# lars-frogner/Impact

Hardware: AMD Instinct MI355X
Metric: voxels stepped/sec + remesh tris/sec, 512^3 grid, 1/2/4/8 MI355X (higher is better)
Workload: dtype i8 voxels, f32 SDF/mesh arithmetic, f64 moments; 1 GPU; config-2 SDF asteroid x2.05 -> 502^3 grid = 512^3 stored voxels (32768 chunks); parallelism=single GPU, voxels_per_gpu=134217728, regions=1, triangles=1813104

## Files before the change

impact_amd/csrc/ivx_api.hip:

```cpp
#include <algorithm>
#include <array>
#include <functional>
#include <cmath>
#include <atomic>
#include <chrono>
#include <cstring>
#include <limits>
#include <map>
#include <unordered_map>
#include <new>
#include <vector>

#include <type_traits>

#include <dlfcn.h>

#include "ivx_internal.hpp"

static thread_local char g_error[512] = "";

void ivx_set_error(const char* fmt, ...) {
    va_list ap;
    va_start(ap, fmt);
    vsnprintf(g_error, sizeof(g_error), fmt, ap);
// ... 602 lines not shown
        g->result_host = nullptr;
    }
    void* ptrs[] = {g->arena, g->positions, g->normals, g->indices, g->index_materials, g->vertex_materials, g->submeshes, g->dev_scratch, g->prog_nodes,
                    g->samp_len, g->samp_ops, g->pairs_dev, g->samp_super, g->probe_points, g->probe_chunk, g->probe_entries};
    for (void* p : ptrs)
        if (p) (void)hipFree(p);
    if (g->host_scratch) (void)hipHostFree(g->host_scratch);
    if (g->result_host) (void)hipHostFree(g->result_host);
    if (g->ev_ready)
        for (int i = 0; i < 2 * IVX_N_TIMED_STAGES; ++i) (void)hipEventDestroy(g->ev[i]);
    delete g;
}

int ivx_grid_upload_dense(ivx_grid* g, const int8_t* sdf, const uint8_t* type, size_t n_voxels) {
    IVX_REQUIRE(g && sdf && type, IVX_ERR_INVALID, "ivx_grid_upload_dense: null argument");
    IVX_REQUIRE(n_voxels == g->n_vox, IVX_ERR_INVALID, "ivx_grid_upload_dense: expected %zu voxels, got %zu", g->n_vox, n_voxels);
    int rc;
    if ((rc = h2d(g, g->sdf, sdf, g->n_vox))) return rc;
    if ((rc = h2d(g, g->type, type, g->n_vox))) return rc;
    if ((rc = ivx_launch_classify(g))) return rc;
    g->mesh_valid = 0;
    g->mesh_built = 0;
    g->occ_ref_valid = 0;
    g->bbox_valid = 0;
    g->regions_valid = 0;
    IVX_HIP_CHECK(ivx_stream_sync(g->ctx->stream));
    return IVX_OK;
}

int ivx_grid_download_dense(ivx_grid* g, int8_t* sdf, uint8_t* type, uint8_t* flags, uint8_t* local_labels, ivx_chunk_info* info, size_t n_voxels) {
// ... 43 lines not shown
        case 5: return g->rparent;
#ifdef IVX_WG_TRACE
        case 6: return g->chunk_moments;
#endif
        case 7: return g->samp_len;
        case 8: return g->samp_ops;
        case 10: return g->sn_hard;
        case 9: return ivx_sn_hard_count(g);
        default: return nullptr;
    }
}

int ivx_sdf_sample(ivx_grid* g, const ivx_sdf_processed_node* nodes, size_t n_nodes, uint32_t stack_size, const uint32_t grid_shape[3],
                   const float shifted_grid_center[3], uint8_t voxel_type) {
    IVX_REQUIRE(g && grid_shape && shifted_grid_center, IVX_ERR_INVALID, "ivx_sdf_sample: null argument");
    IVX_REQUIRE(n_nodes == 0 || nodes, IVX_ERR_INVALID, "ivx_sdf_sample: null node array");
    for (int d = 0; d < 3; ++d) {
        const uint32_t cap = (d == 0 ? g->gx : g->cc[d]) * 16u;
        IVX_REQUIRE(grid_shape[d] <= cap, IVX_ERR_INVALID, "ivx_sdf_sample: grid shape %u exceeds the chunk grid (%u voxels) along axis %d", grid_shape[d], cap, d);
    }
    int depth = 0, max_depth = 0;
    for (size_t i = 0; i < n_nodes; ++i) {
        const uint32_t k = nodes[i].kind;
        IVX_REQUIRE(k <= 9, IVX_ERR_INVALID, "ivx_sdf_sample: unsupported node kind %u", k);
        IVX_REQUIRE(k != 6 || nodes[i].reserved[1] <= 255u, IVX_ERR_INVALID, "ivx_sdf_sample: noise node with more than 255 octaves");
        if (k <= 2) max_depth = std::max(max_depth, ++depth);
        else if (k >= 7) {
            IVX_REQUIRE(depth >= 2, IVX_ERR_INVALID, "ivx_sdf_sample: malformed node program (combination without two operands)");
            --depth;
        } else if (k == 5 || k == 6) {
// ... 11 lines not shown
    }
    rc = ivx_launch_sdf_sample(g, static_cast<const ivx_sdf_processed_node*>(g->dev_scratch), (uint32_t)n_nodes, (uint32_t)max_depth, grid_shape,
                               shifted_grid_center, voxel_type, 0u, false, ivx_sdf_has_noise(nodes, n_nodes));
    if (rc) return rc;
    g->mesh_valid = 0;
    g->mesh_built = 0;
    g->occ_ref_valid = 0;
    g->bbox_valid = 0;
    g->regions_valid = 0;
    IVX_HIP_CHECK(ivx_stream_sync(g->ctx->stream));
    return IVX_OK;
}

int ivx_derive_state(ivx_grid* g) {
    IVX_REQUIRE(g, IVX_ERR_INVALID, "ivx_derive_state: null grid");
    int rc = ivx_launch_derive(g, 0);
    if (rc) return rc;
    g->mesh_valid = 0;
    g->regions_valid = 0;
    IVX_HIP_CHECK(ivx_stream_sync(g->ctx->stream));
    return IVX_OK;
}

int ivx_occupied_ranges(ivx_grid* g, uint32_t out[12]) {
    IVX_REQUIRE(g && out, IVX_ERR_INVALID, "ivx_occupied_ranges: null argument");
    IVX_REQUIRE(g->bbox_valid, IVX_ERR_STATE, "ivx_occupied_ranges: the chunk boxes come from the derive sweep (call ivx_derive_state first)");
    uint32_t* d = g->rscalar + 16;
    int rc;
    if ((rc = ivx_launch_occupied(g, d))) return rc;
    uint32_t raw[12];
    if ((rc = d2h(g, raw, d, 12 * sizeof(uint32_t)))) return rc;
    ivx_occupied_from_raw(g, raw, out);
    memcpy(g->occ_ref, out, sizeof(g->occ_ref));
    g->occ_ref_valid = 1;
    return IVX_OK;
}

int ivx_remesh(ivx_grid* g, ivx_mesh_counts* out) {
    IVX_REQUIRE(g && out, IVX_ERR_INVALID, "ivx_remesh: null argument");
    int rc;
    if ((rc = ivx_launch_sn_count(g))) return rc;
    if ((rc = ivx_launch_sn_scan(g))) return rc;
    uint32_t totals[3];
    if ((rc = d2h(g, totals, g->chunk_offsets + 2 * (size_t)g->n_chunks, sizeof(totals)))) return rc;
    if ((rc = ensure_mesh_capacity(g, totals[0], totals[1], totals[2]))) return rc;
    if (totals[1] > 0 && (rc = ivx_launch_sn_emit(g))) return rc;
    g->mesh_counts.n_vertices = totals[0];
    g->mesh_counts.n_indices = totals[1];
    g->mesh_counts.n_submeshes = totals[2];
    g->mesh_counts.reserved = 0;
    g->mesh_valid = 1;
    g->mesh_built = 1;
    g->mesh_serial += 1;
    *out = g->mesh_counts;
// ... 3 lines not shown

static void ivx_edit_state_free(struct ivx_edit_state* e);
struct ivx_edit_state;
static ivx_edit_state* edit_state(ivx_grid* g);
static bool edit_needs_lookup(ivx_grid* g, uint32_t chunk, uint32_t out3[3]);
static int edit_sync_upload(ivx_grid* g, const void* src, size_t bytes, void* d_dst);
static void edit_sync_mark(ivx_grid* g, int pending);
static int edit_sync_pending(ivx_grid* g);
static bool edit_sync_drained_take(ivx_grid* g);

static int edit_early_needs(ivx_grid* g, const char* who, std::vector<uint32_t>& list);
static int edit_sync_stage(ivx_grid* g, const void* src, size_t bytes, void** dev_view);
static int edit_sync_stage_done(ivx_grid* g);
static int mesh_sync_enqueue(ivx_grid* g, const uint8_t* invalidated_chunks, const char* who) {
    IVX_REQUIRE(g, IVX_ERR_INVALID, "%s: null argument", who);
    ivx_many_other_context other_(g->ctx);
    IVX_REQUIRE(!edit_sync_pending(g), IVX_ERR_STATE, "%s: a sync of this object is in flight (ivx_mesh_sync_collect first)", who);
    IVX_REQUIRE(g->mesh_built, IVX_ERR_STATE, "ivx_mesh_sync: there is no mesh to synchronise (call ivx_remesh first)");
    IVX_REQUIRE(g->regions_valid, IVX_ERR_STATE, "ivx_mesh_sync: derived state must be current (the edit ops leave it so)");
    IVX_REQUIRE(g->x_off == 0 && g->gx == g->cc[0] && !g->has_ghost[0] && !g->has_ghost[1], IVX_ERR_STATE,
                "ivx_mesh_sync: not available on a slab of a decomposed grid");
    int rc;
    static const bool trace_ = getenv("IVX_MANY_TRACE") != nullptr;
    static thread_local double acc_[6];
    static thread_local int calls_ = 0;
    auto tp_ = std::chrono::steady_clock::now();
    auto lap_ = [&](int slot) {
        if (!trace_) return;
        const auto t = std::chrono::steady_clock::now();
        acc_[slot] += 1e-3 * (double)std::chrono::duration_cast<std::chrono::nanoseconds>(t - tp_).count();
// ... 296 lines not shown

static int densities_on_device(ivx_grid* g, const float densities[256], const float** d_out) {
    if (g->has_dens && memcmp(g->dens_host, densities, sizeof(g->dens_host)) == 0) {
        *d_out = g->dens_dev;
        return IVX_OK;
    }
    if (!g->dens_call) IVX_HIP_CHECK(hipMalloc(reinterpret_cast<void**>(&g->dens_call), 256 * sizeof(float)));
    int rc = h2d(g, g->dens_call, densities, 256 * sizeof(float));
    if (rc) return rc;
    *d_out = g->dens_call;
    return IVX_OK;
}

int ivx_inertia(ivx_grid* g, const float densities[256], ivx_moments* out) {
    IVX_REQUIRE(g && densities && out, IVX_ERR_INVALID, "ivx_inertia: null argument");
    double* out_dev = g->partials + g->partial_blocks * 10;
    int rc;
    const float* d_dens = nullptr;
    if ((rc = densities_on_device(g, densities, &d_dens))) return rc;
    if ((rc = ivx_launch_inertia(g, d_dens, out_dev, 0))) return rc;
    if ((rc = d2h(g, out->m64, out_dev, 10 * sizeof(double)))) return rc;
    for (int i = 0; i < 10; ++i) out->m32[i] = (float)out->m64[i];
    out->reserved[0] = out->reserved[1] = 0;
    return IVX_OK;
}

int ivx_label_regions(ivx_grid* g, uint32_t* region_count) {
    IVX_REQUIRE(g && region_count, IVX_ERR_INVALID, "ivx_label_regions: null argument");
    int rc;
    if ((rc = ivx_launch_ccl_local(g, 0))) return rc;
    if ((rc = ivx_launch_ccl_merge(g))) return rc;
    if ((rc = ivx_launch_ccl_resolve(g))) return rc;
    uint32_t sc[2];
    if ((rc = d2h(g, sc, g->rscalar, sizeof(sc)))) return rc;
    IVX_REQUIRE((sc[1] & 1u) == 0, IVX_ERR_CAPACITY,
                "ivx_label_regions: a chunk has more than 254 local regions (the reference's CHUNK_MAX_REGIONS limit, split_detection.rs:145-157)");
    g->region_count = sc[0];
    g->regions_valid = 1;
    *region_count = sc[0];
    return IVX_OK;
}

int ivx_region_labels_download(ivx_grid* g, uint32_t* labels, size_t n_voxels) {
// ... 76 lines not shown
}
static int rederive_collect(ivx_grid* g) {
    ivx_step_result res;
    const int rc = ivx_voxel_step_collect(g, &res);
    if (rc) return rc;
    g->mesh_valid = 0;
    return IVX_OK;
}
static int rederive(ivx_grid* g) {
    const int rc = rederive_enqueue(g);
    return rc ? rc : rederive_collect(g);
}

int ivx_split_off_smallest_region(ivx_grid* parent, ivx_grid** child, uint32_t origin_offset_in_parent[3], int* outcome, ivx_region_desc* moved) {
    IVX_REQUIRE(parent && child && origin_offset_in_parent && outcome, IVX_ERR_INVALID, "ivx_split_off_smallest_region: null argument");
    *child = nullptr;
    *outcome = 0;
    IVX_REQUIRE(parent->regions_valid, IVX_ERR_STATE, "ivx_split_off_smallest_region: call ivx_label_regions first");
    IVX_REQUIRE(parent->x_off == 0 && parent->gx == parent->cc[0] && !parent->has_ghost[0] && !parent->has_ghost[1], IVX_ERR_STATE,
                "ivx_split_off_smallest_region: not available on a slab of a decomposed grid");
    if (parent->region_count < 2) return IVX_OK;
    int rc;
    if (!parent->has_dens) {
        float ones[256];
        for (float& x : ones) x = 1.0f;
        if ((rc = h2d(parent, parent->dens_dev, ones, sizeof(ones)))) return rc;
        memcpy(parent->dens_host, ones, sizeof(ones));
        parent->has_dens = 1;
    }
    std::vector<ivx_region_desc> d;
// ... 44 lines not shown
        return rc;
    }
    if (c && (rc = rederive(c))) {
        ivx_grid_destroy(c);
        return rc;
    }
    *child = c;
    *outcome = c ? 1 : 2;
    return IVX_OK;
}

static int step_enqueue(ivx_grid* g, uint32_t stages, const uint16_t* slab_nbr_ids, void* slab_record, uint32_t part = 3u);
static int ivx_step_collect_launch(ivx_grid* g);
int ivx_split_off_all(ivx_grid* parent, size_t cap, ivx_grid** children, uint32_t* origins3, int* outcomes, ivx_region_desc* moved, size_t* n_out) {
    IVX_REQUIRE(parent && n_out && (cap == 0 || (children && origins3 && outcomes)), IVX_ERR_INVALID, "ivx_split_off_all: null argument");
    *n_out = 0;
    IVX_REQUIRE(parent->regions_valid, IVX_ERR_STATE, "ivx_split_off_all: call ivx_label_regions first");
    IVX_REQUIRE(parent->x_off == 0 && parent->gx == parent->cc[0] && !parent->has_ghost[0] && !parent->has_ghost[1], IVX_ERR_STATE,
                "ivx_split_off_all: not available on a slab of a decomposed grid");
    if (parent->region_count < 2) return IVX_OK;
    const size_t n = parent->region_count - 1u;
    *n_out = n;
    IVX_REQUIRE(n <= cap, IVX_ERR_CAPACITY, "ivx_split_off_all: %zu split-offs exceed capacity %zu", n, cap);
    int rc;
    hipStream_t s = parent->ctx->stream;
    float ones[256];
    for (float& x : ones) x = 1.0f;
    if (!parent->has_dens) {
        if ((rc = h2d(parent, parent->dens_dev, ones, sizeof(ones)))) return rc;
        memcpy(parent->dens_host, ones, sizeof(ones));
// ... 164 lines not shown
        if ((rc = ivx_launch_split_repack(c, single, off))) {
            ivx_grid_destroy(single);
            return rc;
        }
        ivx_grid_destroy(c);
        c = single;
        *pc = c;
        for (int q = 0; q < 3; ++q) origin[q] += off[q];
    }
    return rederive(c);
}

int ivx_clip_polyhedron(ivx_grid* parent, const float* planes4, size_t n_planes, const float aabb[6], int copy, ivx_grid** child,
                        uint32_t origin_offset_in_parent[3], int* outcome) {
    IVX_REQUIRE(parent && planes4 && aabb && child && origin_offset_in_parent && outcome, IVX_ERR_INVALID, "ivx_clip_polyhedron: null argument");
    *child = nullptr;
    *outcome = 0;
    IVX_REQUIRE(n_planes >= 1 && n_planes <= 64, IVX_ERR_CAPACITY, "ivx_clip_polyhedron: 1..64 planes supported, got %zu", n_planes);
    IVX_REQUIRE(parent->regions_valid, IVX_ERR_STATE, "ivx_clip_polyhedron: the object needs its derived state (ivx_derive_state + ivx_label_regions)");
    IVX_REQUIRE(parent->x_off == 0 && parent->gx == parent->cc[0] && !parent->has_ghost[0] && !parent->has_ghost[1], IVX_ERR_STATE,
                "ivx_clip_polyhedron: not available on a slab of a decomposed grid");
    int rc;
    uint32_t* d_occ = parent->rscalar + 16;
    if ((rc = ivx_launch_occupied(parent, d_occ))) return rc;
    uint32_t occ[12], occ_raw[12];
    if ((rc = d2h(parent, occ_raw, d_occ, sizeof(occ_raw)))) return rc;
    ivx_occupied_from_raw(parent, occ_raw, occ);
    if (occ[1] == 0) return IVX_OK;
    uint32_t lo[3], cc[3];
    for (int q = 0; q < 3; ++q) {
// ... 16 lines not shown
        ivx_grid_destroy(c);
        return rc;
    }
    if ((rc = complete_extracted(parent, &c, origin_offset_in_parent))) {
        if (c) ivx_grid_destroy(c);
        return rc;
    }
    *child = c;
    *outcome = c ? 1 : 2;
    return IVX_OK;
}

int ivx_copy_polyhedra(ivx_grid* parent, const float* planes4, const uint32_t* plane_counts, const float* aabbs6, size_t n_sets, ivx_grid** children,
                       uint32_t* origins3, int* outcomes) {
    IVX_REQUIRE(parent && planes4 && plane_counts && aabbs6 && children && origins3 && outcomes, IVX_ERR_INVALID, "ivx_copy_polyhedra: null argument");
    IVX_REQUIRE(parent->regions_valid, IVX_ERR_STATE, "ivx_copy_polyhedra: the object needs its derived state (ivx_derive_state + ivx_label_regions)");
    IVX_REQUIRE(parent->x_off == 0 && parent->gx == parent->cc[0] && !parent->has_ghost[0] && !parent->has_ghost[1], IVX_ERR_STATE,
                "ivx_copy_polyhedra: not available on a slab of a decomposed grid");
    for (size_t f = 0; f < n_sets; ++f) {
        children[f] = nullptr;
        outcomes[f] = 0;
        IVX_REQUIRE(plane_counts[f] >= 1 && plane_counts[f] <= 64, IVX_ERR_CAPACITY, "ivx_copy_polyhedra: 1..64 planes per polyhedron, set %zu has %u", f, plane_counts[f]);
    }
    if (n_sets == 0) return IVX_OK;
    int rc;
    hipStream_t s = parent->ctx->stream;
    uint32_t* d_occ = parent->rscalar + 16;
    if ((rc = ivx_launch_occupied(parent, d_occ))) return rc;
    uint32_t occ[12], occ_raw[12];
    if ((rc = d2h(parent, occ_raw, d_occ, sizeof(occ_raw)))) return rc;
// ... 240 lines not shown
    int rc = ensure_pinned(&e->pinned_up, &e->pinned_up_bytes, bytes);
    if (rc) return rc;
    if (e->pinned_up_bytes != had || !e->pinned_up_dev) IVX_HIP_CHECK(hipHostGetDevicePointer(&e->pinned_up_dev, e->pinned_up, 0));
    memcpy(e->pinned_up, src, bytes);
    *dev_view = e->pinned_up_dev;
    return IVX_OK;
}
static int edit_sync_stage_done(ivx_grid* g) {
    (void)g;
    return IVX_OK;
}

static int absorb_enqueue(ivx_grid* g, const char* who, int capsule, const float center[3], const float seg[3], float influence_radius, float shape_radius,
                          const float densities[256]) {
    IVX_REQUIRE(g && center && densities && (seg || !capsule), IVX_ERR_INVALID, "%s: null argument", who);
    ivx_many_other_context other_(g->ctx);
    IVX_REQUIRE(influence_radius >= 0.0f && shape_radius >= 0.0f, IVX_ERR_INVALID, "%s: negative radius", who);
    IVX_REQUIRE(g->regions_valid, IVX_ERR_STATE, "%s: derived state and regions must be current (ivx_derive_state + ivx_label_regions)", who);
    IVX_REQUIRE(g->x_off == 0 && g->gx == g->cc[0] && !g->has_ghost[0] && !g->has_ghost[1], IVX_ERR_STATE, "%s: not available on a slab of a decomposed grid",
                who);
    ivx_edit_state* e = edit_state(g);
    IVX_REQUIRE(e, IVX_ERR_CAPACITY, "%s: out of host memory", who);
    IVX_REQUIRE(!e->pending, IVX_ERR_STATE, "%s: an edit of this object is in flight (ivx_absorb_collect first)", who);
    int rc;
    uint32_t occ[12];
    if ((rc = reference_occupied(g, occ))) return rc;
    int32_t vlo[3], vhi[3];
    uint32_t lo[3], cc[3];
    e->nothing = 0;
    for (int d = 0; d < 3; ++d) {
// ... 71 lines not shown
    e->early_armed = 0, e->early_taken = 0;
    if (e->staged && g->early_needs_on) {
        e->early_seq += 1u;
        g->post1_needs_early = reinterpret_cast<uint32_t*>(static_cast<char*>(e->pinned_dev) + e->off_early);
        g->post1_needs_counter = reinterpret_cast<uint32_t*>(base + e->off_cnt) + 2;
        g->post1_needs_bell = reinterpret_cast<uint32_t*>(static_cast<char*>(e->pinned_dev) + e->off_bell);
        g->post1_needs_seq = e->early_seq;
        *reinterpret_cast<volatile uint32_t*>(static_cast<char*>(e->pinned) + e->off_bell) = 0u;
        e->early_armed = 1;
    }
    {
        const uint32_t keep = g->stage_timing_off;
        g->stage_timing_off = 0xFFFFFFFFu;
        g->preset_fresh |= IVX_SCRATCH_REGIONS;
        g->regions_labelled_locally = 1;
        rc = ivx_voxel_step_enqueue(g, IVX_STAGE_REGIONS);
        g->regions_labelled_locally = 0;
        g->stage_timing_off = keep;
        if (rc) return rc;
    }
    if (e->staged) {
        g->gather_copy_src = reinterpret_cast<const uint32_t*>(base);
        g->gather_copy_dst = static_cast<uint32_t*>(e->pinned_dev);
        g->gather_copy_words = (uint32_t)(((e->early_armed ? e->off_needs : e->total) + 3) / 4);
    }
    e->pending = 1;
    return IVX_OK;
}

static int absorb_collect(ivx_grid* g, const char* who, ivx_absorb_result* out, uint32_t* emptied_by_type, uint8_t* invalidated_chunks) {
    IVX_REQUIRE(g && out, IVX_ERR_INVALID, "%s: null argument", who);
// ... 1012 lines not shown
             if ((r = ivx_launch_mutual_pass(q.a, q.b, &p.pass[0], nullptr, d_offsets, list_dev + out_offsets[i], counts[i], 1))) return r;
             return ivx_launch_mutual_pass(q.b, q.a, &p.pass[1], nullptr, d_offsets + p.wg_a, list_dev + out_offsets[i], counts[i], 1);
         })))
        return rc;
    IVX_HIP_CHECK(ivx_stream_sync(s));
    memcpy(out, c->pinned_scratch, run * sizeof(ivx_contact));
    return IVX_OK;
}

int ivx_absorb_mutual(ivx_grid* a, const float rotation_a[4], const float translation_a[3], const float densities_a[256], ivx_grid* b, const float rotation_b[4],
                      const float translation_b[3], const float densities_b[256], float smoothness, ivx_absorb_result* out_a, ivx_absorb_result* out_b,
                      uint8_t* invalidated_chunks_a, uint8_t* invalidated_chunks_b) {
    const char* who = "ivx_absorb_mutual";
    IVX_REQUIRE(a && b && rotation_a && translation_a && densities_a && rotation_b && translation_b && densities_b && out_a && out_b, IVX_ERR_INVALID,
                "%s: null argument", who);
    IVX_REQUIRE(a != b && a->ctx == b->ctx, IVX_ERR_INVALID, "%s: two different objects of one context are needed", who);
    IVX_REQUIRE(smoothness >= 0.0f, IVX_ERR_INVALID, "%s: negative smoothness", who);
    for (ivx_grid* g : {a, b}) {
        IVX_REQUIRE(g->regions_valid, IVX_ERR_STATE, "%s: derived state and regions must be current (ivx_derive_state + ivx_label_regions)", who);
        IVX_REQUIRE(g->x_off == 0 && g->gx == g->cc[0] && !g->has_ghost[0] && !g->has_ghost[1], IVX_ERR_STATE,
                    "%s: not available on a slab of a decomposed grid", who);
    }
    memset(out_a, 0, sizeof(*out_a));
    memset(out_b, 0, sizeof(*out_b));
    if (invalidated_chunks_a) memset(invalidated_chunks_a, 0, a->n_chunks);
    if (invalidated_chunks_b) memset(invalidated_chunks_b, 0, b->n_chunks);
    int rc;
    uint32_t occ_a[12], occ_b[12];
    if ((rc = reference_occupied(a, occ_a))) return rc;
    if ((rc = reference_occupied(b, occ_b))) return rc;
// ... 164 lines not shown
    g->vt_noise_freq = noise_frequency;
    g->vt_type_freq = voxel_type_frequency;
    g->vt_seed = seed;
    return IVX_OK;
}

int ivx_grid_set_densities(ivx_grid* g, const float densities[256]) {
    IVX_REQUIRE(g && densities, IVX_ERR_INVALID, "ivx_grid_set_densities: null argument");
    memcpy(g->dens_host, densities, sizeof(g->dens_host));
    if (!ivx_many_upload(g->ctx, g, g->dens_dev, g->dens_host, sizeof(g->dens_host)))
        IVX_HIP_CHECK(ivx_memcpy_async(g->dens_dev, g->dens_host, sizeof(g->dens_host), hipMemcpyHostToDevice, g->ctx->stream));
    g->has_dens = 1;
    return IVX_OK;
}

static int ensure_pairs(ivx_grid* g);
static int step_enqueue(ivx_grid* g, uint32_t stages, const uint16_t* slab_nbr_ids, void* slab_record, uint32_t part) {
    IVX_REQUIRE(g, IVX_ERR_INVALID, "ivx_voxel_step_enqueue: null grid");
    const bool front = (part & 1u) != 0u, back = (part & 2u) != 0u;
    ivx_many_other_context other_(g->ctx);
    IVX_REQUIRE(!(stages & IVX_STAGE_SAMPLE) || g->prog_n > 0, IVX_ERR_STATE, "ivx_voxel_step: no SDF program resident (ivx_grid_set_sdf_program)");
    IVX_REQUIRE(!(stages & IVX_STAGE_INERTIA) || g->has_dens, IVX_ERR_STATE, "ivx_voxel_step: no densities resident (ivx_grid_set_densities)");
    hipStream_t s = g->ctx->stream;
    g->ahead_unordered_ok = g->pending_stages == 0;
    g->results_in_block = 0;
    if (!g->ev_ready) {
        for (int i = 0; i < 2 * IVX_N_TIMED_STAGES; ++i) IVX_HIP_CHECK(hipEventCreate(&g->ev[i]));
        g->ev_ready = 1;
    }
    if (!g->result_host) {
        IVX_HIP_CHECK(hipHostMalloc(reinterpret_cast<void**>(&g->result_host), 64 * sizeof(uint32_t), hipHostMallocMapped));
        memset(g->result_host, 0, 64 * sizeof(uint32_t));
        IVX_HIP_CHECK(hipHostGetDevicePointer(reinterpret_cast<void**>(&g->result_host_dev), g->result_host, 0));
    }
    int rc;
    if (stages & IVX_STAGE_SAMPLE)
        if ((rc = ivx_sampler_buffers(g))) return rc;
    uint32_t preset_in_sample = 0, preset_in_derive = 0;
    if (front) {
        uint32_t need = 0;
// ... 70 lines not shown
        if ((rc = ivx_launch_step_post2(g, post, slab_nbr_ids))) return rc;
        T1(3);
        if (post & (IVX_STAGE_REGIONS | IVX_STAGE_REMESH)) {
            T0(4);
            if (fused_assign) {
                if ((rc = ivx_launch_step_emit(g, post, (post & IVX_STAGE_REGIONS) != 0, slab_record, slab_nbr_ids != nullptr))) return rc;
                if (slab_record) g->results_in_block = 1;
            } else {
                if ((post & IVX_STAGE_REMESH) && (rc = ivx_launch_step_emit(g, IVX_STAGE_REMESH))) return rc;
                if ((post & IVX_STAGE_REGIONS) && (rc = ivx_launch_ccl_resolve(g))) return rc;
            }
            T1(4);
        }
        if (!g->ahead_unordered_ok && (rc = ivx_sampler_launch_ahead(g, true))) return rc;
        if ((post & IVX_STAGE_REGIONS) && fused_assign) {
            T0(5);
            if ((rc = ivx_launch_step_assign(g, (post & IVX_STAGE_REMESH) != 0))) return rc;
            T1(5);
        }
        if (post & IVX_STAGE_REMESH) {
            g->mesh_valid = 0;
            g->scratch_dirty |= IVX_SCRATCH_SN;
        }
        if (post & IVX_STAGE_REGIONS) g->scratch_dirty |= IVX_SCRATCH_REGIONS;
    }
#undef T0
#undef T1
    if (back && (rc = ivx_sampler_launch_ahead(g, !g->ahead_unordered_ok))) return rc;
    g->pending_stages |= stages;
    return IVX_OK;
}

int ivx_voxel_step_enqueue(ivx_grid* g, uint32_t stages) { return step_enqueue(g, stages, nullptr, nullptr); }
// ... 27 lines not shown
    IVX_REQUIRE(g, IVX_ERR_INVALID, "ivx_grid_set_stage_timing: null grid");
    g->stage_timing_off = ~slot_mask;
    return IVX_OK;
}

static uint64_t collect_spin_ns() {
    static const uint64_t ns = [] {
        const char* e = getenv("IVX_COLLECT_SPIN_US");
        const long us = e ? strtol(e, nullptr, 10) : 2000;
        return (uint64_t)(us < 0 ? 0 : us) * 1000ull;
    }();
    return ns;
}

static int ivx_step_collect_launch(ivx_grid* g) {
    if (g->results_in_block || g->gather_launched) return IVX_OK;
    if (!g->result_host) {
        IVX_HIP_CHECK(hipHostMalloc(reinterpret_cast<void**>(&g->result_host), 64 * sizeof(uint32_t), hipHostMallocMapped));
        memset(g->result_host, 0, 64 * sizeof(uint32_t));
        IVX_HIP_CHECK(hipHostGetDevicePointer(reinterpret_cast<void**>(&g->result_host_dev), g->result_host, 0));
    }
    g->gather_flush_id = ivx_many_flush_count();
    const int rc = ivx_launch_step_gather(g);
    if (!rc) g->gather_launched = 1;
    return rc;
}

int ivx_voxel_step_collect(ivx_grid* g, ivx_step_result* out) {
    IVX_REQUIRE(g && out, IVX_ERR_INVALID, "ivx_voxel_step_collect: null argument");
    ivx_many_other_context other_(g->ctx);
    hipStream_t s = g->ctx->stream;
    memset(out, 0, sizeof(*out));
    const uint32_t stages = g->pending_stages;
    if (!g->result_host) {
        IVX_HIP_CHECK(hipHostMalloc(reinterpret_cast<void**>(&g->result_host), 64 * sizeof(uint32_t), hipHostMallocMapped));
        memset(g->result_host, 0, 64 * sizeof(uint32_t));
        IVX_HIP_CHECK(hipHostGetDevicePointer(reinterpret_cast<void**>(&g->result_host_dev), g->result_host, 0));
    }
    const bool have_results = g->results_in_block != 0;
    g->results_in_block = 0;
    if (!have_results) {
        if (!g->gather_launched) {
            int rc = ivx_launch_step_gather(g);
            if (rc) return rc;
            (void)ivx_many_break();
        }
        if (g->gather_launched && ivx_many_recording() && g->gather_flush_id == ivx_many_flush_count()) (void)ivx_many_break();
        g->gather_launched = 0;
    } else if (hipStreamQuery(s) != hipSuccess) {
        IVX_HIP_CHECK(ivx_stream_sync(s));
    }
    if (!have_results) {
        const volatile uint32_t* bell = g->result_host + 63;
        const uint32_t want = g->result_seq;
        const uint64_t budget_ns = collect_spin_ns();
        bool rung = false;
// ... 56 lines not shown
        g->mesh_counts.n_indices = totals[1];
        g->mesh_counts.n_submeshes = totals[2];
        g->mesh_counts.reserved = 0;
        g->mesh_growth_pending = grown_later ? 1 : 0;
        if (!grown_later) {
            g->mesh_valid = 1;
            g->mesh_built = 1;
            g->mesh_serial += 1;
        }
    }
    if (stages & IVX_STAGE_INERTIA) {
        memcpy(out->moments.m64, sc + 32, 10 * sizeof(double));
        for (int i = 0; i < 10; ++i) out->moments.m32[i] = (float)out->moments.m64[i];
    }
    out->mesh = g->mesh_counts;
    for (int i = 0; i < IVX_N_TIMED_STAGES; ++i) {
        float ms = 0.0f;
        if ((g->timed_mask >> i) & 1u)
            if (hipEventElapsedTime(&ms, *g->ev_start_ref[i], g->ev[2 * i + 1]) != hipSuccess) ms = 0.0f;
        out->stage_ms[i] = ms;
    }
    g->pending_stages = 0;
    g->timed_mask = 0;
    return IVX_OK;
}

int ivx_voxel_step(ivx_grid* g, uint32_t stages, ivx_step_result* out) {
    IVX_REQUIRE(g && out, IVX_ERR_INVALID, "ivx_voxel_step: null argument");
    int rc = ivx_voxel_step_enqueue(g, stages);
    if (rc) return rc;
// ... 65 lines not shown
    rc = ivx_launch_face_pairs(g, side, static_cast<const uint16_t*>(neighbour_face_labels), g->pairs_dev, g->pairs_dev + 4 + 128, IVX_MAX_FACE_PAIRS,
                               g->pairs_dev + 4);
    if (rc) return rc;
    g->pairs_enqueued = 1;
    return IVX_OK;
}

size_t ivx_step_record_words(void) { return 28 + 2 * (size_t)IVX_MAX_FACE_PAIRS; }

int ivx_step_record_enqueue(ivx_grid* g, void* device_record) {
    IVX_REQUIRE(g && device_record, IVX_ERR_INVALID, "ivx_step_record_enqueue: null argument");
    int rc = ensure_pairs(g);
    if (rc) return rc;
    rc = ivx_launch_step_record(g, g->pairs_enqueued ? g->pairs_dev : nullptr, g->pairs_dev + 4 + 128, IVX_MAX_FACE_PAIRS, device_record, g->result_host_dev != nullptr);
    if (!rc && g->result_host_dev) g->results_in_block = 1;
    g->pairs_enqueued = 0;
    return rc;
}

int ivx_many_begin(ivx_ctx* c);
int ivx_many_flush(ivx_ctx* c);
static int many_check(ivx_grid* const* grids, size_t n, const char* who) {
    IVX_REQUIRE(grids && grids[0], IVX_ERR_INVALID, "%s: null object list", who);
    static thread_local std::vector<const ivx_grid*> seen;
    seen.assign(grids, grids + n);
    std::sort(seen.begin(), seen.end());
    for (size_t i = 0; i < n; ++i) {
        IVX_REQUIRE(grids[i] && grids[i]->ctx == grids[0]->ctx, IVX_ERR_INVALID, "%s: object %zu is null or belongs to another context", who, i);
        IVX_REQUIRE(i == 0 || seen[i] != seen[i - 1], IVX_ERR_INVALID, "%s: an object is listed twice", who);
    }
// ... 195 lines not shown
```

impact_amd/csrc/ivx_internal.hpp:

```cpp
#pragma once
#include <hip/hip_runtime.h>

#include <cstdarg>
#include <cstdint>
#include <cstdio>
#include <cstring>

#include "../../include/impact_voxel_hip.h"
#include "many.hpp"

static inline hipError_t ivx_memset_async(void* p, int v, size_t n, hipStream_t s) {
    (void)ivx_many_break();
    return hipMemsetAsync(p, v, n, s);
}
static inline hipError_t ivx_memcpy_async(void* d, const void* src, size_t n, hipMemcpyKind k, hipStream_t s) {
    (void)ivx_many_break();
    return hipMemcpyAsync(d, src, n, k, s);
}
static inline hipError_t ivx_stream_sync(hipStream_t s) {
    (void)ivx_many_break();
    return hipStreamSynchronize(s);
}
static inline hipError_t ivx_memcpy_sync(void* d, const void* src, size_t n, hipMemcpyKind k) {
    (void)ivx_many_break();
// ... 154 lines not shown
    hipEvent_t ahead_go, ahead_done;
    uint32_t* samp_super;
    size_t samp_super_words;
    hipEvent_t ev[2 * IVX_N_TIMED_STAGES];
    int ev_ready;
    uint32_t* result_host;
    uint32_t* result_host_dev;
    uint32_t result_seq;
    hipEvent_t* ev_start_ref[IVX_N_TIMED_STAGES];
    uint32_t pending_stages;
    uint32_t timed_mask;
    uint32_t* pairs_dev;
    unsigned long long* record_head_copy;
    uint32_t record_head_words;
    int results_in_block;
    int pairs_enqueued;
    int pairs_zeroed;
    uint32_t preset_ahead, preset_fresh;
    void* host_scratch;
    size_t host_scratch_bytes;
    float* probe_points;
    uint32_t* probe_chunk;
    uint32_t* probe_entries;
    size_t probe_point_cap, probe_entry_cap;
    uint32_t n_probe_points, n_probe_sub;
    uint64_t mesh_serial, probes_serial;
    ivx_block* mesh_block;
    uint32_t mesh_pooled;
    int defer_mesh_growth;
    int mesh_growth_pending;
// ... 106 lines not shown
static inline uint32_t ivx_list_grid(const ivx_grid* g) {
    uint32_t n = g->last_active ? g->last_active + g->last_active / 8u + 64u : (uint32_t)g->ctx->n_cu * 32u;
    const uint32_t lo = (g->n_chunks + 255u) / 256u;
    if (n > g->n_chunks) n = g->n_chunks;
    return n < lo ? lo : n;
}

static inline bool ivx_has_interior_planes(const ivx_grid* g) { return (int)g->cc[0] - (g->has_ghost[0] ? 1 : 0) - (g->has_ghost[1] ? 1 : 0) > 0; }
static inline uint32_t* ivx_wc(const ivx_grid* g) { return g->work_counts + g->wc_cur; }
static inline void ivx_planes_touched(ivx_grid* g) {
    g->signs_current = 0;
    g->needs_current = 0;
}
#define IVX_SCRATCH_EVAL_ROLL 8u
#define IVX_SCRATCH_REGIONS 1u
#define IVX_SCRATCH_SN 2u
#define IVX_SN_TAIL_WORDS 288u
#define IVX_SN_GROUP_WORDS 32u
#define IVX_SCRATCH_EVAL 4u

static inline GridView ivx_view(const ivx_grid* g) {
    GridView v;
    v.cx = g->cc[0];
    v.cy = g->cc[1];
    v.cz = g->cc[2];
    v.sdf = g->sdf;
    v.type = g->type;
    v.signs = g->chunk_signs;
    v.kface = g->kface;
#ifdef IVX_WG_TRACE
// ... 21 lines not shown
                          bool resident_program = false, bool noise = false);
bool ivx_sdf_has_noise(const ivx_sdf_processed_node* nodes, size_t n);
#define IVX_PART_REGIONS 1u
#define IVX_PART_MOMENTS 2u
int ivx_launch_derive(ivx_grid* g, uint32_t parts, uint32_t preset_groups = 0);
int ivx_launch_derive_box(ivx_grid* g, uint32_t parts, const uint32_t lo[3], const uint32_t cc[3], uint32_t* d_out_list);
int ivx_ensure_active_list(ivx_grid* g);
int ivx_ensure_dense(ivx_grid* g);
int ivx_launch_step_preset(ivx_grid* g, uint32_t groups);
static inline void ivx_step_preset_ahead(ivx_grid* g, uint32_t groups) { g->preset_ahead |= groups; }
int ivx_voxel_step_enqueue_part(ivx_grid* g, uint32_t stages, uint32_t part);
int ivx_launch_halo_pack_parts(ivx_grid* g, void* buf_lo, void* buf_hi, uint32_t what);
int ivx_launch_step_post1(ivx_grid* g, uint32_t stages);
int ivx_launch_step_post2(ivx_grid* g, uint32_t stages, const uint16_t* face_pair_ids = nullptr);
int ivx_launch_step_emit(ivx_grid* g, uint32_t stages, bool general_in_assign = false, void* slab_record = nullptr, bool record_has_pairs = false);
int ivx_launch_step_assign(ivx_grid* g, bool with_mesher_general = false, bool with_ccl = true);
int ivx_launch_step_gather(ivx_grid* g);
bool ivx_step_assign_fits(const ivx_grid* g);
int ivx_sampler_buffers(ivx_grid* g);
int ivx_sampler_ahead_cancel(ivx_grid* g);
void ivx_sampler_ahead_free(ivx_grid* g);
int ivx_sampler_launch_ahead(ivx_grid* g, bool behind_stream);
void ivx_sdf_annotate_host(ivx_sdf_processed_node* nodes, size_t n);
int ivx_launch_occupied(ivx_grid* g, uint32_t* d_raw);
void ivx_occupied_from_raw(const ivx_grid* g, const uint32_t raw[12], uint32_t out[12]);
int ivx_launch_sn_count(ivx_grid* g);
int ivx_launch_list_mesh_needs(ivx_grid* g, uint32_t n, const uint32_t* d_list, uint32_t* d_out);
int ivx_launch_box_mesh_needs(ivx_grid* g, const uint32_t t_lo[3], const uint32_t t_cc[3], const uint32_t b_lo[3], const uint32_t b_cc[3], const uint32_t* d_touched,
                              uint32_t* d_out);
int ivx_launch_sn_scan(ivx_grid* g);
int ivx_launch_sn_emit(ivx_grid* g);
// ... 43 lines not shown
```

impact_amd/csrc/slab_comm.cpp:

```cpp
#include <dlfcn.h>
#include <fcntl.h>
#include <sys/mman.h>
#include <sys/stat.h>
#include <unistd.h>

#include <algorithm>
#include <atomic>
#include <chrono>
#include <cstdlib>
#include <cstdio>
#include <cstring>
#include <thread>
#include <vector>

#include "ivx_internal.hpp"

namespace {

constexpr size_t HEAD_PAIRS = 64;
constexpr size_t HEAD_WORDS = 28 + 2 * HEAD_PAIRS;

typedef struct ncclComm* ncclComm_t;
struct ncclUniqueId_ {
    char internal[128];
// ... 608 lines not shown
            if (m->ipc_peer_recv[s] && !m->ipc_peer_same_process[s]) (void)hipIpcCloseMemHandle(m->ipc_peer_recv[s]);
        munmap(m->ipc, sizeof(IpcShared));
        if (m->rank == 0) (void)shm_unlink(m->ipc_name);
    }
    delete m;
}

int ivx_slab_create(ivx_comm* m, ivx_grid* g, int rank, ivx_slab** out) {
    IVX_REQUIRE(m && g && out && rank >= 0 && rank < m->nranks && (m->rank < 0 || rank == m->rank), IVX_ERR_INVALID, "ivx_slab_create: bad argument");
    IVX_REQUIRE(g->ctx == m->ctx, IVX_ERR_INVALID, "ivx_slab_create: grid and communicator belong to different contexts");
    *out = nullptr;
    ivx_slab* sl = new (std::nothrow) ivx_slab();
    IVX_REQUIRE(sl, IVX_ERR_CAPACITY, "ivx_slab_create: out of host memory");
    sl->comm = m;
    sl->grid = g;
    sl->rank = rank;
    sl->halo_bytes = ivx_halo_bytes(g);
    sl->face_bytes = ivx_region_face_bytes(g);
    sl->rec_words = ivx_step_record_words();
    sl->has_lo = rank > 0;
    sl->has_hi = rank + 1 < m->nranks;
    sl->enqueued = 0;
    sl->map_offset = 0;
    sl->local_err = IVX_OK;
    const size_t msg = (sl->halo_bytes + sl->face_bytes + 255) & ~(size_t)255;
    bool ok = true;
    for (int s = 0; s < 2; ++s) {
        ok = ok && hipMalloc(reinterpret_cast<void**>(&sl->send[s]), msg) == hipSuccess;
        ok = ok && hipMalloc(reinterpret_cast<void**>(&sl->recv[s]), msg) == hipSuccess;
        sl->send2[s] = nullptr;
// ... 351 lines not shown
```

impact_amd/csrc/step_fused.hip:

```cpp
#include "ccl_roles.hpp"
#include "sn_roles.hpp"
#include "table_roles.hpp"
#include "many.hpp"

namespace {
using namespace ivx_roles;

struct StepArgs {
    GridView g;
    float extent;
    uint32_t x_off;
    uint32_t n_chunks;
    uint32_t nb[6];
    const uint8_t* flags;
    uint8_t* labels;
    ivx_chunk_info* info;
    uint32_t* rparent;
    uint32_t* rcompid;
    uint32_t* rscalar;
    uint32_t* multi_list;
    uint32_t* ccl_group_sums;
    const uint8_t* touch;
    uint32_t* counts;
    uint32_t* sn_group_sums;
// ... 9 lines not shown
    uint4* vmats;
    uint32_t* hard_count;
    uint32_t* hard_list;
    sn::SnWalk walk;
    ivx_submesh* submeshes;
    uint32_t vcap, icap, scap;
    const uint32_t* bbox;
    uint32_t* occ_part;
    uint32_t n_occ_slots;
    const float* dens;
    const double* chunk_moments;
    double* partials;
    uint32_t n_partials;
    double* moments_out;
    uint32_t* host_block;
    const uint32_t* eval_count;
    uint32_t count_run;
    uint32_t x_part;
    uint32_t seq;
    uint32_t fp_side, fp_cap;
    const uint16_t* fp_nbr;
    uint32_t* fp_count;
    uint2* fp_pairs;
    uint32_t* fp_seen;
    unsigned long long* record;
    uint32_t record_max_pairs;
    unsigned long long* record_head;
    uint32_t record_head_words;
    sn::BoxNeeds needs_box;
    const uint32_t* needs_touched;
// ... 127 lines not shown
    }
    b -= a.nb[1];
    if (b < a.nb[2]) {
        role_step_record(a.rscalar, a.fp_count, a.fp_pairs, a.offsets + 2 * (size_t)a.n_chunks, a.moments_out, a.x_off, a.record_max_pairs, a.record);
        if (a.record_head) {
            __syncthreads();
            for (uint32_t i = threadIdx.x; i < a.record_head_words; i += 256u) a.record_head[i] = a.record[i];
        }
        if (threadIdx.x < 64u) role_result_gather(a.rscalar, a.offsets + 2 * (size_t)a.n_chunks, a.moments_out, a.work_count, a.eval_count, a.host_block, false, 0u);
    }
}
template <bool ST>
__global__ __launch_bounds__(256) __attribute__((amdgpu_waves_per_eu(ST ? IVX_EMIT_ST_PER_CU : 4, ST ? IVX_EMIT_ST_PER_CU : 4))) void k_step_emit(StepArgs a) { step_emit_body<ST>(a, blockIdx.x, gridDim.x); }
IVX_MANY_TWIN(k_step_emit_many, StepArgs, step_emit_body<false>, __launch_bounds__(256) __attribute__((amdgpu_waves_per_eu(4, 4))))

__device__ __forceinline__ void step_assign_body(const StepArgs& a, uint32_t b, uint32_t) {
    if (b < a.nb[0]) {
        role_ccl_assign<true>(b, a.nb[0], a.g, a.rparent, a.multi_list , a.ccl_group_sums, a.nb[0], a.rcompid, a.rscalar);
        return;
    }
    sn::role_sn_emit_general<false>(b - a.nb[0], a.nb[1], sn_params(a), a.positions, a.normals, a.indices, a.imats, a.vmats, a.submeshes,
                                    a.offsets + 2 * (size_t)a.n_chunks + 2, a.emit_items, a.vcap, a.icap, a.scap, nullptr, a.hard_count, a.hard_list);
}
__global__ __launch_bounds__(256) __attribute__((amdgpu_waves_per_eu(4, 4))) void k_step_assign(StepArgs a) { step_assign_body(a, blockIdx.x, gridDim.x); }
IVX_MANY_TWIN(k_step_assign_many, StepArgs, step_assign_body, __launch_bounds__(256) __attribute__((amdgpu_waves_per_eu(4, 4))))

__device__ __forceinline__ void step_gather_body(const StepArgs& a, uint32_t, uint32_t) {
    role_result_gather(a.rscalar, a.offsets + 2 * (size_t)a.n_chunks, a.moments_out, a.work_count, a.eval_count, a.host_block, false, 0u);
    for (uint32_t i0 = threadIdx.x; i0 < a.copy_words; i0 += 512u) {
        uint32_t v[8];
#pragma unroll
        for (uint32_t q = 0; q < 8u; ++q) v[q] = i0 + 64u * q < a.copy_words ? a.copy_src[i0 + 64u * q] : 0u;
#pragma unroll
        for (uint32_t q = 0; q < 8u; ++q)
            if (i0 + 64u * q < a.copy_words) a.copy_dst[i0 + 64u * q] = v[q];
    }
    __threadfence_system();
// ... 174 lines not shown
        a.record_head = g->record_head_copy;
        a.record_head_words = g->record_head_words;
        a.nb[2] = 1;
    }
    const uint32_t total = a.nb[0] + a.nb[1] + a.nb[2];
    if (total == 0) return IVX_OK;
    if (single_type) IVX_KLAUNCH(k_step_emit<true>, dim3(total), dim3(256), 0, g->ctx->stream, a);
    else if (!ivx_many_try(g->ctx, g, IVX_MK_EMIT, total, a)) IVX_KLAUNCH(k_step_emit<false>, dim3(total), dim3(256), 0, g->ctx->stream, a);
    IVX_HIP_CHECK(hipGetLastError());
    if ((stages & IVX_STAGE_REMESH) && !general_in_assign) return ivx_launch_sn_emit_general(g);
    return IVX_OK;
}

bool ivx_step_assign_fits(const ivx_grid* g) { return (g->n_chunks + 255u) / 256u <= ASSIGN_MAX_GROUPS; }

int ivx_launch_step_assign(ivx_grid* g, bool with_mesher_general, bool with_ccl) {
    StepArgs a = make_args(g);
    a.nb[0] = with_ccl ? (g->n_chunks + 255u) / 256u : 0u;
    a.nb[1] = with_mesher_general ? sn::ivx_emit_general_grid(g, g->n_chunks) : 0u;
    if (a.nb[0] + a.nb[1] == 0u) return IVX_OK;
    if (!ivx_many_try(g->ctx, g, IVX_MK_ASSIGN, a.nb[0] + a.nb[1], a)) IVX_KLAUNCH(k_step_assign, dim3(a.nb[0] + a.nb[1]), dim3(256), 0, g->ctx->stream, a);
    IVX_HIP_CHECK(hipGetLastError());
    return IVX_OK;
}

int ivx_launch_step_gather(ivx_grid* g) {
    StepArgs a = make_args(g);
    a.seq = ++g->result_seq;
    a.copy_src = g->gather_copy_src, a.copy_dst = g->gather_copy_dst, a.copy_words = g->gather_copy_words;
    g->gather_copy_words = 0;
    if (!ivx_many_try(g->ctx, g, IVX_MK_GATHER, 1u, a)) IVX_KLAUNCH(k_step_gather, dim3(1), dim3(64), 0, g->ctx->stream, a);
    IVX_HIP_CHECK(hipGetLastError());
    return IVX_OK;
}

#ifdef IVX_WG_TRACE
extern "C" int ivx_debug_exact_trace(unsigned long long* out512) {
    return hipMemcpyFromSymbol(out512, HIP_SYMBOL(ivx_exact_trace_buf), 512 * sizeof(unsigned long long)) == hipSuccess ? 0 : -1;
}
#endif
```

Before: 843.3 billion voxels/s.

## Fold result gather into assign kernel via last-block ticket tail

Each block of the fused assign kernel increments a device-scope ticket when it finishes. The last block to arrive runs the result gather itself and publishes the sequence number to the host block, so the separate single-block gather kernel launch is no longer needed on the common single-GPU path. Every other API entry point drops the in-flight tail flag, and slabs and region-only enqueues opt out. In exchange there are extra fences and atomics per block. The ticket reset writes to the host block index rather than the rscalar ticket slot, which could leave the counter stale unless rscalar is cleared elsewhere.

```diff
diff --git a/impact_amd/csrc/ivx_api.hip b/impact_amd/csrc/ivx_api.hip
--- a/impact_amd/csrc/ivx_api.hip
+++ b/impact_amd/csrc/ivx_api.hip
@@ -640,6 +640,7 @@
 
 int ivx_grid_upload_dense(ivx_grid* g, const int8_t* sdf, const uint8_t* type, size_t n_voxels) {
     IVX_REQUIRE(g && sdf && type, IVX_ERR_INVALID, "ivx_grid_upload_dense: null argument");
+    ivx_step_tail_drop(g);
     IVX_REQUIRE(n_voxels == g->n_vox, IVX_ERR_INVALID, "ivx_grid_upload_dense: expected %zu voxels, got %zu", g->n_vox, n_voxels);
     int rc;
     if ((rc = h2d(g, g->sdf, sdf, g->n_vox))) return rc;
@@ -713,6 +714,7 @@
 int ivx_sdf_sample(ivx_grid* g, const ivx_sdf_processed_node* nodes, size_t n_nodes, uint32_t stack_size, const uint32_t grid_shape[3],
                    const float shifted_grid_center[3], uint8_t voxel_type) {
     IVX_REQUIRE(g && grid_shape && shifted_grid_center, IVX_ERR_INVALID, "ivx_sdf_sample: null argument");
+    ivx_step_tail_drop(g);
     IVX_REQUIRE(n_nodes == 0 || nodes, IVX_ERR_INVALID, "ivx_sdf_sample: null node array");
     for (int d = 0; d < 3; ++d) {
         const uint32_t cap = (d == 0 ? g->gx : g->cc[d]) * 16u;
@@ -754,6 +756,7 @@
 
 int ivx_derive_state(ivx_grid* g) {
     IVX_REQUIRE(g, IVX_ERR_INVALID, "ivx_derive_state: null grid");
+    ivx_step_tail_drop(g);
     int rc = ivx_launch_derive(g, 0);
     if (rc) return rc;
     g->mesh_valid = 0;
@@ -764,6 +767,7 @@
 
 int ivx_occupied_ranges(ivx_grid* g, uint32_t out[12]) {
     IVX_REQUIRE(g && out, IVX_ERR_INVALID, "ivx_occupied_ranges: null argument");
+    ivx_step_tail_drop(g);
     IVX_REQUIRE(g->bbox_valid, IVX_ERR_STATE, "ivx_occupied_ranges: the chunk boxes come from the derive sweep (call ivx_derive_state first)");
     uint32_t* d = g->rscalar + 16;
     int rc;
@@ -778,6 +782,7 @@
 
 int ivx_remesh(ivx_grid* g, ivx_mesh_counts* out) {
     IVX_REQUIRE(g && out, IVX_ERR_INVALID, "ivx_remesh: null argument");
+    ivx_step_tail_drop(g);
     int rc;
     if ((rc = ivx_launch_sn_count(g))) return rc;
     if ((rc = ivx_launch_sn_scan(g))) return rc;
@@ -811,6 +816,7 @@
 static int edit_sync_stage_done(ivx_grid* g);
 static int mesh_sync_enqueue(ivx_grid* g, const uint8_t* invalidated_chunks, const char* who) {
     IVX_REQUIRE(g, IVX_ERR_INVALID, "%s: null argument", who);
+    ivx_step_tail_drop(g);
     ivx_many_other_context other_(g->ctx);
     IVX_REQUIRE(!edit_sync_pending(g), IVX_ERR_STATE, "%s: a sync of this object is in flight (ivx_mesh_sync_collect first)", who);
     IVX_REQUIRE(g->mesh_built, IVX_ERR_STATE, "ivx_mesh_sync: there is no mesh to synchronise (call ivx_remesh first)");
@@ -1137,6 +1143,7 @@
 
 int ivx_inertia(ivx_grid* g, const float densities[256], ivx_moments* out) {
     IVX_REQUIRE(g && densities && out, IVX_ERR_INVALID, "ivx_inertia: null argument");
+    ivx_step_tail_drop(g);
     double* out_dev = g->partials + g->partial_blocks * 10;
     int rc;
     const float* d_dens = nullptr;
@@ -1150,6 +1157,7 @@
 
 int ivx_label_regions(ivx_grid* g, uint32_t* region_count) {
     IVX_REQUIRE(g && region_count, IVX_ERR_INVALID, "ivx_label_regions: null argument");
+    ivx_step_tail_drop(g);
     int rc;
     if ((rc = ivx_launch_ccl_local(g, 0))) return rc;
     if ((rc = ivx_launch_ccl_merge(g))) return rc;
@@ -1256,6 +1264,7 @@
 
 int ivx_split_off_smallest_region(ivx_grid* parent, ivx_grid** child, uint32_t origin_offset_in_parent[3], int* outcome, ivx_region_desc* moved) {
     IVX_REQUIRE(parent && child && origin_offset_in_parent && outcome, IVX_ERR_INVALID, "ivx_split_off_smallest_region: null argument");
+    ivx_step_tail_drop(parent);
     *child = nullptr;
     *outcome = 0;
     IVX_REQUIRE(parent->regions_valid, IVX_ERR_STATE, "ivx_split_off_smallest_region: call ivx_label_regions first");
@@ -1330,6 +1339,7 @@
 static int ivx_step_collect_launch(ivx_grid* g);
 int ivx_split_off_all(ivx_grid* parent, size_t cap, ivx_grid** children, uint32_t* origins3, int* outcomes, ivx_region_desc* moved, size_t* n_out) {
     IVX_REQUIRE(parent && n_out && (cap == 0 || (children && origins3 && outcomes)), IVX_ERR_INVALID, "ivx_split_off_all: null argument");
+    ivx_step_tail_drop(parent);
     *n_out = 0;
     IVX_REQUIRE(parent->regions_valid, IVX_ERR_STATE, "ivx_split_off_all: call ivx_label_regions first");
     IVX_REQUIRE(parent->x_off == 0 && parent->gx == parent->cc[0] && !parent->has_ghost[0] && !parent->has_ghost[1], IVX_ERR_STATE,
@@ -1524,6 +1534,7 @@
 int ivx_clip_polyhedron(ivx_grid* parent, const float* planes4, size_t n_planes, const float aabb[6], int copy, ivx_grid** child,
                         uint32_t origin_offset_in_parent[3], int* outcome) {
     IVX_REQUIRE(parent && planes4 && aabb && child && origin_offset_in_parent && outcome, IVX_ERR_INVALID, "ivx_clip_polyhedron: null argument");
+    ivx_step_tail_drop(parent);
     *child = nullptr;
     *outcome = 0;
     IVX_REQUIRE(n_planes >= 1 && n_planes <= 64, IVX_ERR_CAPACITY, "ivx_clip_polyhedron: 1..64 planes supported, got %zu", n_planes);
@@ -1570,6 +1581,7 @@
 int ivx_copy_polyhedra(ivx_grid* parent, const float* planes4, const uint32_t* plane_counts, const float* aabbs6, size_t n_sets, ivx_grid** children,
                        uint32_t* origins3, int* outcomes) {
     IVX_REQUIRE(parent && planes4 && plane_counts && aabbs6 && children && origins3 && outcomes, IVX_ERR_INVALID, "ivx_copy_polyhedra: null argument");
+    ivx_step_tail_drop(parent);
     IVX_REQUIRE(parent->regions_valid, IVX_ERR_STATE, "ivx_copy_polyhedra: the object needs its derived state (ivx_derive_state + ivx_label_regions)");
     IVX_REQUIRE(parent->x_off == 0 && parent->gx == parent->cc[0] && !parent->has_ghost[0] && !parent->has_ghost[1], IVX_ERR_STATE,
                 "ivx_copy_polyhedra: not available on a slab of a decomposed grid");
@@ -1840,6 +1852,7 @@
 static int absorb_enqueue(ivx_grid* g, const char* who, int capsule, const float center[3], const float seg[3], float influence_radius, float shape_radius,
                           const float densities[256]) {
     IVX_REQUIRE(g && center && densities && (seg || !capsule), IVX_ERR_INVALID, "%s: null argument", who);
+    ivx_step_tail_drop(g);
     ivx_many_other_context other_(g->ctx);
     IVX_REQUIRE(influence_radius >= 0.0f && shape_radius >= 0.0f, IVX_ERR_INVALID, "%s: negative radius", who);
     IVX_REQUIRE(g->regions_valid, IVX_ERR_STATE, "%s: derived state and regions must be current (ivx_derive_state + ivx_label_regions)", who);
@@ -1941,7 +1954,10 @@
         g->stage_timing_off = 0xFFFFFFFFu;
         g->preset_fresh |= IVX_SCRATCH_REGIONS;
         g->regions_labelled_locally = 1;
+        const int keep_tail = g->step_tail_off;
+        g->step_tail_off = 1;
         rc = ivx_voxel_step_enqueue(g, IVX_STAGE_REGIONS);
+        g->step_tail_off = keep_tail;
         g->regions_labelled_locally = 0;
         g->stage_timing_off = keep;
         if (rc) return rc;
@@ -2984,6 +3000,8 @@
     const char* who = "ivx_absorb_mutual";
     IVX_REQUIRE(a && b && rotation_a && translation_a && densities_a && rotation_b && translation_b && densities_b && out_a && out_b, IVX_ERR_INVALID,
                 "%s: null argument", who);
+    ivx_step_tail_drop(a);
+    ivx_step_tail_drop(b);
     IVX_REQUIRE(a != b && a->ctx == b->ctx, IVX_ERR_INVALID, "%s: two different objects of one context are needed", who);
     IVX_REQUIRE(smoothness >= 0.0f, IVX_ERR_INVALID, "%s: negative smoothness", who);
     for (ivx_grid* g : {a, b}) {
@@ -3178,6 +3196,15 @@
     return IVX_OK;
 }
 
+static bool step_tail_on() {
+    static const bool on = [] {
+        const char* e = getenv("IVX_STEP_TAIL");
+        return !e || atoi(e) != 0;
+    }();
+    return on;
+}
+static bool step_tail_holds(const ivx_grid* g) { return g->tail_in_flight && g->gather_copy_words == 0u; }
+
 static int ensure_pairs(ivx_grid* g);
 static int step_enqueue(ivx_grid* g, uint32_t stages, const uint16_t* slab_nbr_ids, void* slab_record, uint32_t part) {
     IVX_REQUIRE(g, IVX_ERR_INVALID, "ivx_voxel_step_enqueue: null grid");
@@ -3188,6 +3215,7 @@
     hipStream_t s = g->ctx->stream;
     g->ahead_unordered_ok = g->pending_stages == 0;
     g->results_in_block = 0;
+    ivx_step_tail_drop(g);
     if (!g->ev_ready) {
         for (int i = 0; i < 2 * IVX_N_TIMED_STAGES; ++i) IVX_HIP_CHECK(hipEventCreate(&g->ev[i]));
         g->ev_ready = 1;
@@ -3288,9 +3316,12 @@
         }
         if (!g->ahead_unordered_ok && (rc = ivx_sampler_launch_ahead(g, true))) return rc;
         if ((post & IVX_STAGE_REGIONS) && fused_assign) {
+            const bool tail = step_tail_on() && !g->step_tail_off && !ivx_many_recording() && !slab_record && part == 3u && !g->has_ghost[0] && !g->has_ghost[1] &&
+                              g->gather_copy_words == 0u;
             T0(5);
-            if ((rc = ivx_launch_step_assign(g, (post & IVX_STAGE_REMESH) != 0))) return rc;
+            if ((rc = ivx_launch_step_assign(g, (post & IVX_STAGE_REMESH) != 0, true, tail))) return rc;
             T1(5);
+            g->tail_in_flight = tail ? 1 : 0;
         }
         if (post & IVX_STAGE_REMESH) {
             g->mesh_valid = 0;
@@ -3348,7 +3379,7 @@
 }
 
 static int ivx_step_collect_launch(ivx_grid* g) {
-    if (g->results_in_block || g->gather_launched) return IVX_OK;
+    if (g->results_in_block || g->gather_launched || step_tail_holds(g)) return IVX_OK;
     if (!g->result_host) {
         IVX_HIP_CHECK(hipHostMalloc(reinterpret_cast<void**>(&g->result_host), 64 * sizeof(uint32_t), hipHostMallocMapped));
         memset(g->result_host, 0, 64 * sizeof(uint32_t));
@@ -3373,7 +3404,9 @@
     }
     const bool have_results = g->results_in_block != 0;
     g->results_in_block = 0;
-    if (!have_results) {
+    const bool in_tail = !have_results && !g->gather_launched && step_tail_holds(g);
+    ivx_step_tail_drop(g);
+    if (!have_results && !in_tail) {
         if (!g->gather_launched) {
             int rc = ivx_launch_step_gather(g);
             if (rc) return rc;
@@ -3460,6 +3493,7 @@
         for (int i = 0; i < 10; ++i) out->moments.m32[i] = (float)out->moments.m64[i];
     }
     out->mesh = g->mesh_counts;
+    if (in_tail && ((g->timed_mask >> 5) & 1u)) IVX_HIP_CHECK(hipEventSynchronize(g->ev[2 * 5 + 1]));
     for (int i = 0; i < IVX_N_TIMED_STAGES; ++i) {
         float ms = 0.0f;
         if ((g->timed_mask >> i) & 1u)
@@ -3555,6 +3589,7 @@
     if (rc) return rc;
     rc = ivx_launch_step_record(g, g->pairs_enqueued ? g->pairs_dev : nullptr, g->pairs_dev + 4 + 128, IVX_MAX_FACE_PAIRS, device_record, g->result_host_dev != nullptr);
     if (!rc && g->result_host_dev) g->results_in_block = 1;
+    ivx_step_tail_drop(g);
     g->pairs_enqueued = 0;
     return rc;
 }
diff --git a/impact_amd/csrc/ivx_internal.hpp b/impact_amd/csrc/ivx_internal.hpp
--- a/impact_amd/csrc/ivx_internal.hpp
+++ b/impact_amd/csrc/ivx_internal.hpp
@@ -192,6 +192,8 @@
     unsigned long long* record_head_copy;
     uint32_t record_head_words;
     int results_in_block;
+    int tail_in_flight;
+    int step_tail_off;
     int pairs_enqueued;
     int pairs_zeroed;
     uint32_t preset_ahead, preset_fresh;
@@ -328,6 +330,7 @@
 }
 #define IVX_SCRATCH_EVAL_ROLL 8u
 #define IVX_SCRATCH_REGIONS 1u
+#define IVX_RSCALAR_TAIL_TICKET 4u
 #define IVX_SCRATCH_SN 2u
 #define IVX_SN_TAIL_WORDS 288u
 #define IVX_SN_GROUP_WORDS 32u
@@ -379,7 +382,8 @@
 int ivx_launch_step_post1(ivx_grid* g, uint32_t stages);
 int ivx_launch_step_post2(ivx_grid* g, uint32_t stages, const uint16_t* face_pair_ids = nullptr);
 int ivx_launch_step_emit(ivx_grid* g, uint32_t stages, bool general_in_assign = false, void* slab_record = nullptr, bool record_has_pairs = false);
-int ivx_launch_step_assign(ivx_grid* g, bool with_mesher_general = false, bool with_ccl = true);
+int ivx_launch_step_assign(ivx_grid* g, bool with_mesher_general = false, bool with_ccl = true, bool tail = false);
+static inline void ivx_step_tail_drop(ivx_grid* g) { g->tail_in_flight = 0; }
 int ivx_launch_step_gather(ivx_grid* g);
 bool ivx_step_assign_fits(const ivx_grid* g);
 int ivx_sampler_buffers(ivx_grid* g);
diff --git a/impact_amd/csrc/slab_comm.cpp b/impact_amd/csrc/slab_comm.cpp
--- a/impact_amd/csrc/slab_comm.cpp
+++ b/impact_amd/csrc/slab_comm.cpp
@@ -646,6 +646,7 @@
     IVX_REQUIRE(sl, IVX_ERR_CAPACITY, "ivx_slab_create: out of host memory");
     sl->comm = m;
     sl->grid = g;
+    g->step_tail_off = 1;
     sl->rank = rank;
     sl->halo_bytes = ivx_halo_bytes(g);
     sl->face_bytes = ivx_region_face_bytes(g);
diff --git a/impact_amd/csrc/step_fused.hip b/impact_amd/csrc/step_fused.hip
--- a/impact_amd/csrc/step_fused.hip
+++ b/impact_amd/csrc/step_fused.hip
@@ -47,6 +47,7 @@
     uint32_t n_partials;
     double* moments_out;
     uint32_t* host_block;
+    uint32_t* tail_ticket;
     const uint32_t* eval_count;
     uint32_t count_run;
     uint32_t x_part;
@@ -204,13 +205,37 @@
 __global__ __launch_bounds__(256) __attribute__((amdgpu_waves_per_eu(ST ? IVX_EMIT_ST_PER_CU : 4, ST ? IVX_EMIT_ST_PER_CU : 4))) void k_step_emit(StepArgs a) { step_emit_body<ST>(a, blockIdx.x, gridDim.x); }
 IVX_MANY_TWIN(k_step_emit_many, StepArgs, step_emit_body<false>, __launch_bounds__(256) __attribute__((amdgpu_waves_per_eu(4, 4))))
 
+__device__ __forceinline__ void step_tail_arrive(const StepArgs& a, uint32_t expected) {
+    asm volatile("s_waitcnt vmcnt(0)" ::: "memory");
+    __syncthreads();
+    if (threadIdx.x >= 64u) return;
+    uint32_t last = 0u;
+    if (threadIdx.x == 0u) {
+        __builtin_amdgcn_fence(__ATOMIC_RELEASE, "agent");
+        asm volatile("s_waitcnt vmcnt(0)" ::: "memory");
+        last = __hip_atomic_fetch_add(a.tail_ticket, 1u, __ATOMIC_RELAXED, __HIP_MEMORY_SCOPE_AGENT) + 1u == expected ? 1u : 0u;
+    }
+    if (!__builtin_amdgcn_readfirstlane(last)) return;
+    __builtin_amdgcn_fence(__ATOMIC_ACQUIRE, "agent");
+    asm volatile("s_waitcnt vmcnt(0)" ::: "memory");
+    role_result_gather(a.rscalar, a.offsets + 2 * (size_t)a.n_chunks, a.moments_out, a.work_count, a.eval_count, a.host_block, false, 0u);
+    if (threadIdx.x == IVX_RSCALAR_TAIL_TICKET) a.host_block[IVX_RSCALAR_TAIL_TICKET] = 0u;
+    __threadfence_system();
+    if (threadIdx.x == 0u) __hip_atomic_store(a.host_block + 63, a.seq, __ATOMIC_RELEASE, __HIP_MEMORY_SCOPE_SYSTEM);
+}
+
 __device__ __forceinline__ void step_assign_body(const StepArgs& a, uint32_t b, uint32_t) {
+    const uint32_t n_hard = a.tail_ticket && a.nb[1] ? a.hard_count[0] : 0u;
+    const uint32_t expected = a.nb[0] + (n_hard ? a.nb[1] : 0u);
     if (b < a.nb[0]) {
         role_ccl_assign<true>(b, a.nb[0], a.g, a.rparent, a.multi_list , a.ccl_group_sums, a.nb[0], a.rcompid, a.rscalar);
-        return;
-    }
+        if (a.tail_ticket) step_tail_arrive(a, expected);
+        return;
+    }
+    if (a.tail_ticket && !n_hard) return;
     sn::role_sn_emit_general<false>(b - a.nb[0], a.nb[1], sn_params(a), a.positions, a.normals, a.indices, a.imats, a.vmats, a.submeshes,
                                     a.offsets + 2 * (size_t)a.n_chunks + 2, a.emit_items, a.vcap, a.icap, a.scap, nullptr, a.hard_count, a.hard_list);
+    if (a.tail_ticket) step_tail_arrive(a, expected);
 }
 __global__ __launch_bounds__(256) __attribute__((amdgpu_waves_per_eu(4, 4))) void k_step_assign(StepArgs a) { step_assign_body(a, blockIdx.x, gridDim.x); }
 IVX_MANY_TWIN(k_step_assign_many, StepArgs, step_assign_body, __launch_bounds__(256) __attribute__((amdgpu_waves_per_eu(4, 4))))
@@ -415,17 +440,22 @@
 
 bool ivx_step_assign_fits(const ivx_grid* g) { return (g->n_chunks + 255u) / 256u <= ASSIGN_MAX_GROUPS; }
 
-int ivx_launch_step_assign(ivx_grid* g, bool with_mesher_general, bool with_ccl) {
+int ivx_launch_step_assign(ivx_grid* g, bool with_mesher_general, bool with_ccl, bool tail) {
     StepArgs a = make_args(g);
     a.nb[0] = with_ccl ? (g->n_chunks + 255u) / 256u : 0u;
     a.nb[1] = with_mesher_general ? sn::ivx_emit_general_grid(g, g->n_chunks) : 0u;
     if (a.nb[0] + a.nb[1] == 0u) return IVX_OK;
+    if (tail) {
+        a.tail_ticket = g->rscalar + IVX_RSCALAR_TAIL_TICKET;
+        a.seq = ++g->result_seq;
+    }
     if (!ivx_many_try(g->ctx, g, IVX_MK_ASSIGN, a.nb[0] + a.nb[1], a)) IVX_KLAUNCH(k_step_assign, dim3(a.nb[0] + a.nb[1]), dim3(256), 0, g->ctx->stream, a);
     IVX_HIP_CHECK(hipGetLastError());
     return IVX_OK;
 }
 
 int ivx_launch_step_gather(ivx_grid* g) {
+    ivx_step_tail_drop(g);
     StepArgs a = make_args(g);
     a.seq = ++g->result_seq;
     a.copy_src = g->gather_copy_src, a.copy_dst = g->gather_copy_dst, a.copy_words = g->gather_copy_words;
```

Measured after the change: 812.8 billion voxels/s. -3.6%, worse.
